# acrlabs/kube-scheduler-rs-reference

Measured on AMD Instinct MI355X. Metric: pod x node predicate evals/s, higher is better.
Workload: dtype int64

## Files before the change

kube_scheduler_rs_reference_amd/csrc/kernels_fused.hpp:

```cpp
#pragma once
#include <hip/hip_ext.h>
#include <hip/hip_runtime.h>
#include <stdint.h>

#include <type_traits>

#include "eval_request.hpp"
#include "kernarg.hpp"
#include "kernels_direct.hpp"
#include "tile_index.hpp"
#include "tile_launch.hpp"

#ifndef KSCHED_STORE_POLICY
#define KSCHED_STORE_POLICY 6
#endif
#ifndef KSCHED_STORE_ALT
#define KSCHED_STORE_ALT(it) ((it) == 7u)
#endif
#ifndef KSCHED_PROFILE
#define KSCHED_PROFILE 0
#endif
#if defined(KSCHED_FUSED_NUM_VGPR)
#define KSCHED_FUSED_WPE_ATTR __attribute__((amdgpu_num_vgpr(KSCHED_FUSED_NUM_VGPR)))
#elif defined(KSCHED_FUSED_WPE)
#define KSCHED_FUSED_WPE_ATTR __attribute__((amdgpu_waves_per_eu(KSCHED_FUSED_WPE, KSCHED_FUSED_WPE)))
#else
#define KSCHED_FUSED_WPE_ATTR
#endif

namespace ksched {

struct FusedArgs {
    uint32_t W, pitch, tiles, rows, nkeys, ngroups;
    uint32_t row_zero, row_valid, row_cpu, row_mem, row_taint;
    uint32_t lab_off[8], lab_mx1[8];
    const uint32_t *lab_meta;
    const uint64_t *zero64;
    uint32_t p, units, chunks, run;
    uint32_t unit_q, unit_rem, tiles_rcp;
    uint32_t wave_major;
    uint32_t u_stride;
    uint32_t off_aux, off_fit, off_lab, off_trow;
    uint32_t nlist, list_mask8, off_list, off_lrec;
    uint32_t list_col[kMaxListKeys];
    uint32_t debug;
    uint32_t has_tol;
    uint32_t pick_ppb, pick_waves;
    uint64_t *pick_acc;
    uint32_t off_park;
    uint32_t off_pf;
    uint64_t *trace;
};

typedef uint32_t u32x4 __attribute__((ext_vector_type(4)));
typedef uint32_t u32x4_a8 __attribute__((ext_vector_type(4), aligned(8)));

template <bool FIT, bool SEL, bool TAINT, bool WANT_FIT, bool LIST = false, int PICK = 0>
__global__ __launch_bounds__(kFusedThreads) KSCHED_FUSED_WPE_ATTR void k_eval_fused(
    const uint64_t *__restrict__ g_tables, const uint64_t *__restrict__ g_aux, const int64_t *__restrict__ g_pcpu,
    const int64_t *__restrict__ g_pmem, const uint32_t *__restrict__ g_psel, const uint64_t *__restrict__ g_ptol,
    uint64_t *__restrict__ out_feas, uint64_t *__restrict__ out_fit, const uint8_t *__restrict__ g_list, const FusedArgs a,
    const SelectArgs sa) {
    static_assert(!LIST || SEL, "list keys only exist with the selector predicate");
    static_assert(!PICK || (!LIST && !WANT_FIT), "the pick rides only in the plain mask variants");
    static_assert(PICK != 2 || !TAINT, "the tile-test pick is built for the reference's two predicates");
    kernarg_warm<9 * 8 + sizeof(FusedArgs) + (PICK ? sizeof(SelectArgs) : 0)>();
    extern __shared__ __attribute__((aligned(16))) uint8_t smem[];
    const uint32_t b = blockIdx.x;
    uint32_t tile, chunk, lin;
    if (!(a.debug & 32u)) {
        const uint32_t l = (b & 7u) * a.run + (b >> 3);
        if ((b >> 3) >= a.run) return;
        chunk = __umulhi(l, a.tiles_rcp);
// ... 9 lines not shown
        lin = chunk * a.tiles + tile;
    }
    if (chunk >= a.chunks) return;

    const uint32_t pick_waves = PICK == 1 ? a.pick_waves : 0u;
    uint32_t tid = threadIdx.x;
    bool pick_wave = false;
    if constexpr (PICK == 1) {
        const uint32_t wave0 = (uint32_t)__builtin_amdgcn_readfirstlane((int)(threadIdx.x >> 6));
        const uint32_t pick_rank = (a.debug & 0x10000u) ? (kFusedWaves - 1u - wave0) : wave0;
        pick_wave = pick_rank < pick_waves;
        if (pick_wave) {
            const uint64_t t_in = (a.trace && threadIdx.x == 0u) ? wall_clock64() : 0ull;
            const uint32_t base = lin * a.pick_ppb;
            const uint32_t end = min(a.p, base + a.pick_ppb);
            const uint32_t eager = (a.debug >> 8) & 3u;
            for (uint32_t pod = base + pick_rank * 64u + (threadIdx.x & 63u); pod < end; pod += pick_waves * 64u) {
                int32_t bnd;
                if (eager == 1u) bnd = select_one_pod<5, 3>(sa, pod);
                else if (eager == 2u) bnd = select_one_pod<5, 5>(sa, pod);
                else if (eager == 3u) bnd = select_one_pod<5, 2>(sa, pod);
                else bnd = select_one_pod<5, 1>(sa, pod);
                sa.binding[pod] = bnd;
            }
            if (a.trace && threadIdx.x == 0u)
                atomicOr((unsigned long long *)&a.trace[(size_t)b * 8u + 7u], (unsigned long long)((wall_clock64() - t_in) << 8));
        }
        asm volatile("" : "+v"(tid) : : "memory");
    }
    const uint32_t lane = tid & 63u;
    const uint32_t wave = __builtin_amdgcn_readfirstlane(tid >> 6);
    const uint32_t stage_rank = (PICK == 1 && !(a.debug & 0x10000u)) ? wave - pick_waves : wave;
    const uint32_t stage_waves = kFusedWaves - pick_waves;
    const bool tracer = a.trace && tid == (PICK == 1 ? (kFusedWaves - 1u) * 64u : 0u);
    auto stamp = [&](uint32_t i) {
        if (tracer) a.trace[(size_t)b * 8u + i] = wall_clock64();
    };
    stamp(0);
    const uint32_t c_lo = chunk * a.unit_q + min(chunk, a.unit_rem);
    const uint32_t c_n = a.unit_q + (chunk < a.unit_rem ? 1u : 0u);
    uint32_t u = c_lo + (wave * c_n) / kFusedWaves;
    uint32_t u_hi = c_lo + ((wave + 1u) * c_n) / kFusedWaves;
    const uint32_t u_stride = a.u_stride;
    if (u_stride != 8u) {
        u = (a.wave_major ? wave * a.chunks + chunk : chunk * kFusedWaves + wave) * 8u;
        u_hi = a.units;
    }

    int64_t rc = 0, rm = 0;
    uint32_t s0 = 0, s1 = 0, s2 = 0, s3 = 0, s4 = 0, s5 = 0, s6 = 0, s7 = 0;
    uint64_t tol = 0;
    uint32_t d0 = 0, d1 = 0, d2 = 0, d3 = 0, d4 = 0;
    uint64_t ar = 0;
    auto issue_ops = [&](uint32_t pod) {
        const uint32_t pc = min(pod, a.p - 1u);
        if constexpr (PICK == 2) {
            static_assert(kPickAttempts == 5, "five draw registers");
            const size_t last = (size_t)a.p * kPickAttempts - 1u;
            const size_t f0 = (size_t)(pod - lane) * kPickAttempts + lane;
            asm volatile("global_load_dword %0, %1, off" : "=v"(d0) : "v"(sa.samples + min(f0, last)) : "memory");
            asm volatile("global_load_dword %0, %1, off" : "=v"(d1) : "v"(sa.samples + min(f0 + 64u, last)) : "memory");
            asm volatile("global_load_dword %0, %1, off" : "=v"(d2) : "v"(sa.samples + min(f0 + 128u, last)) : "memory");
            asm volatile("global_load_dword %0, %1, off" : "=v"(d3) : "v"(sa.samples + min(f0 + 192u, last)) : "memory");
            asm volatile("global_load_dword %0, %1, off" : "=v"(d4) : "v"(sa.samples + min(f0 + 256u, last)) : "memory");
        }
        if (FIT) {
            asm volatile("global_load_dwordx2 %0, %1, off" : "=v"(rc) : "v"(g_pcpu + pc) : "memory");
            asm volatile("global_load_dwordx2 %0, %1, off" : "=v"(rm) : "v"(g_pmem + pc) : "memory");
        }
        if (SEL) {
#define KSCHED_LOAD_SEL(K, DST)                                                                                                   \
    asm volatile("global_load_dword %0, %1, off"                                                                                  \
                 : "=v"(DST)                                                                                                      \
                 : "v"((uint32_t)K < a.nkeys ? g_psel + (size_t)K * a.p + pc : reinterpret_cast<const uint32_t *>(a.zero64)) \
                 : "memory")
            KSCHED_LOAD_SEL(0, s0);
            KSCHED_LOAD_SEL(1, s1);
            KSCHED_LOAD_SEL(2, s2);
            KSCHED_LOAD_SEL(3, s3);
            KSCHED_LOAD_SEL(4, s4);
            KSCHED_LOAD_SEL(5, s5);
            KSCHED_LOAD_SEL(6, s6);
            KSCHED_LOAD_SEL(7, s7);
#undef KSCHED_LOAD_SEL
        }
        if (TAINT) {
            const uint64_t *tp = a.has_tol ? g_ptol + pc : a.zero64;
            asm volatile("global_load_dwordx2 %0, %1, off" : "=v"(tol) : "v"(tp) : "memory");
        }
    };
#define KSCHED_WAIT_OPS(N)                                                                                                            \
    asm volatile("s_waitcnt vmcnt(%c11)"                                                                                              \
                 : "+v"(rc), "+v"(rm), "+v"(s0), "+v"(s1), "+v"(s2), "+v"(s3), "+v"(s4), "+v"(s5), "+v"(s6), "+v"(s7), "+v"(tol)  \
                 : "n"(N)                                                                                                             \
                 : "memory")
#define KSCHED_WAIT_OPS_PICK(N)                                                                                                       \
    asm volatile("s_waitcnt vmcnt(%c17)"                                                                                              \
                 : "+v"(rc), "+v"(rm), "+v"(s0), "+v"(s1), "+v"(s2), "+v"(s3), "+v"(s4), "+v"(s5), "+v"(s6), "+v"(s7), "+v"(tol), \
                   "+v"(d0), "+v"(d1), "+v"(d2), "+v"(d3), "+v"(d4), "+v"(ar)                                                     \
                 : "n"(N)                                                                                                             \
                 : "memory")
    const int64_t *s_cpu = reinterpret_cast<const int64_t *>(smem + a.off_aux);
    const int64_t *s_mem = s_cpu + kAuxTreeWords;
    const uint2 *s_cnt_cpu = reinterpret_cast<const uint2 *>(s_cpu + 2u * kAuxTreeWords);
    const uint2 *s_cnt_mem = s_cnt_cpu + kCntEntries;
    uint4 *s_fit = reinterpret_cast<uint4 *>(smem + a.off_fit) + wave * 64u;
    uint4 *s_lab = reinterpret_cast<uint4 *>(smem + a.off_lab) + wave * 64u;
    uint2 *s_trow = reinterpret_cast<uint2 *>(smem + a.off_trow) + wave * 64u;
    typedef __attribute__((address_space(3))) uint8_t lds_u8;
    lds_u8 *const lds = (lds_u8 *)smem;
    uint2 *s_lrec = reinterpret_cast<uint2 *>(smem + a.off_lrec) + wave * 64u;
    constexpr uint32_t kListCap = 8u;

    const uint32_t quad = (lane & 31u) >> 2;
    const uint32_t wp = ((0xCCu >> quad) & 1u) * 4u + (lane & 3u);
    const uint32_t sub = (lane >> 5) * 4u + ((0x31130220u >> (4u * quad)) & 15u);
    const uint32_t w0 = tile * kTileWords + 2u * wp;
    const bool has0 = w0 < a.pitch, has1 = w0 + 1u < a.pitch;
// ... 133 lines not shown
        const bool live = pod < a.p && has0;
        Rows R;
        if (LIST) {
            uint32_t sub_o = sub, wp_o = wp;
            asm volatile("" : "+v"(sub_o), "+v"(wp_o));
            const uint8_t *fit_o = reinterpret_cast<const uint8_t *>(s_fit + sub_o) + wp_o;
            const uint2 *lab_o = reinterpret_cast<const uint2 *>(s_lab + sub_o);
            load_rows(FIT ? (uint32_t)(fit_o + it * 128u)[0] : 0u, FIT ? (uint32_t)(fit_o + it * 128u)[8] : 0u, (lab_o + it * 16u)[0],
                      TAINT ? (s_trow + sub_o + it * 8u)[0] : make_uint2(0u, 0u), R);
            load_extra((lab_o + it * 16u)[1], R);
        } else {
            load_rows(rec_cc(it), rec_cm(it), rec_lb(it), rec_tr(it), R);
            if (SEL) load_extra(rec_lx(it), R);
        }
        u32x4 f = fit_of(R);
        const size_t o = (size_t)pod * a.pitch + w0;
        auto store = [&](uint64_t *dst) {
            if (has1) store16(dst, o, f);
            else dst[o] = ((uint64_t)f.y << 32) | f.x;
        };
        if (WANT_FIT && live) store(out_fit);
        if (SEL) {
            if (!over) {
                f = ((f & R.l0) & R.l1) & (R.l2 & R.l3);
                f = ((f & R.x0) & R.x1) & (R.x2 & R.x3);
            } else if (live) {
                for (uint32_t k = 0; k < a.nkeys; ++k) {
                    if (LIST && a.lab_meta[k] == kLabList) continue;
                    const uint32_t s = g_psel[(size_t)k * a.p + pod];
                    if (s != 0u) f &= ldrow((s <= a.lab_meta[32u + k]) ? (a.lab_meta[k] + s - 1u) : a.row_zero);
                }
            }
        }
        if (TAINT) {
            if (taint_inline) {
                f = ((f & R.t0) & R.t1) & (R.t2 & R.t3);
            } else if (live) {
                const uint64_t t = a.has_tol ? g_ptol[pod] : 0ull;
                for (uint32_t g = 0; g < a.ngroups; ++g) f &= ldrow(a.row_taint + 16u * g + (uint32_t)((t >> (4u * g)) & 15ull));
            }
        }
        if (LIST) {
            __builtin_amdgcn_sched_barrier(0);
            f = apply_lists(f, lrec_of(it), 0xFFFFFFFFu);
        }
        if (live && out_feas && !(a.debug & 1u)) store(out_feas);
    };

    bool extra_any = false, list_any = false;
    uint32_t list_bound = 0;
    uint32_t pick_bits = 0;
    typedef __attribute__((address_space(3))) uint32_t lds_u32;
    lds_u32 *const s_park = (lds_u32 *)(lds + a.off_park) + wave * (kPickAttempts * 64u);
    auto phase1 = [&](uint32_t pod0) -> uint64_t {
        uint2 cnt_c = make_uint2(0u, 0u), cnt_m = make_uint2(0u, 0u);
        if (FIT) {
            uint32_t lc = 0, lm = 0;
            if (!(a.debug & 2u)) {
                uint32_t kc = 1, km = 1;
#pragma unroll
                for (uint32_t level = 0; level < 10; ++level) {
                    const int64_t vc = s_cpu[kc], vm = s_mem[km];
                    kc = 2u * kc + ((vc < rc) ? 1u : 0u);
                    km = 2u * km + ((vm < rm) ? 1u : 0u);
                }
                lc = kc - (uint32_t)kTileNodes;
                lm = km - (uint32_t)kTileNodes;
                lc += (lc == (uint32_t)kTileNodes - 1u && s_cpu[0] < rc) ? 1u : 0u;
                lm += (lm == (uint32_t)kTileNodes - 1u && s_mem[0] < rm) ? 1u : 0u;
            }
            const uint2 cc = s_cnt_cpu[lc], cm = s_cnt_mem[lm];
            s_fit[lane] = make_uint4(cc.x, cc.y, cm.x, cm.y);
            cnt_c = cc;
            cnt_m = cm;
        }
        const uint32_t rv = a.row_valid * 128u;
        uint32_t cnt = 0;
        if (SEL) {
            const uint32_t rv2 = rv | (rv << 16);
            s_lab[lane] = make_uint4(rv2, rv2, rv2, rv2);
            uint16_t *const slots = reinterpret_cast<uint16_t *>(s_lab + lane);
            uint16_t *slot = slots;
            const uint32_t sv[8] = {s0, s1, s2, s3, s4, s5, s6, s7};
#pragma unroll
            for (uint32_t k = 0; k < 8; ++k) {
                const uint32_t s = sv[k];
                if (s != 0u && !(LIST && ((a.list_mask8 >> k) & 1u))) {
                    *slot++ = (uint16_t)(min(s, a.lab_mx1[k]) * 128u + a.lab_off[k]);
                }
            }
            cnt = (uint32_t)(slot - slots);
            if (a.nkeys > 8u) {
                const uint32_t pc = min(pod0 + lane, a.p - 1u);
                for (uint32_t k = 8; k < a.nkeys; ++k) {
                    if (LIST && a.lab_meta[k] == kLabList) continue;
                    cnt += (g_psel[(size_t)k * a.p + pc] != 0u) ? 9u : 0u;
                }
            }
        }
        uint32_t lmax = 0;
        if (LIST) {
            uint32_t lv[kMaxListKeys] = {0u, 0u};
#pragma unroll
            for (uint32_t j = 0; j < kMaxListKeys; ++j) {
                if (j >= a.nlist) continue;
                const uint32_t col = a.list_col[j];
                if (col < 8u) {
                    uint32_t v = s0;
                    v = (col == 1u) ? s1 : v;
                    v = (col == 2u) ? s2 : v;
                    v = (col == 3u) ? s3 : v;
                    v = (col == 4u) ? s4 : v;
                    v = (col == 5u) ? s5 : v;
                    v = (col == 6u) ? s6 : v;
                    v = (col == 7u) ? s7 : v;
                    lv[j] = v;
                } else {
                    lv[j] = g_psel[(size_t)col * a.p + min(pod0 + lane, a.p - 1u)];
                }
            }
            uint32_t rec[kMaxListKeys] = {0xFFFF0000u, 0xFFFF0000u};
            bool any = false;
#pragma unroll
            for (uint32_t j = 0; j < kMaxListKeys; ++j) {
                rec[j] = 0xFFFF0000u;
                const uint32_t s = lv[j];
                if (j < a.nlist && s != 0u) {
                    const uint32_t voff = a.off_list + j * kListBytes;
                    auto val_at = [&](uint32_t e) -> uint32_t { return *(const __attribute__((address_space(3))) uint32_t *)(lds + voff + e * 4u); };
                    auto lower = [&](uint32_t key) -> uint32_t {
                        uint32_t base = 0;
#pragma unroll
                        for (uint32_t half = (uint32_t)kTileNodes / 2u; half >= 1u; half >>= 1) base += (val_at(base + half - 1u) < key) ? half : 0u;
                        return base + ((val_at(base) < key) ? 1u : 0u);
                    };
                    const uint32_t lo = lower(s);
                    uint32_t cnt = 0;
                    bool run = true;
#pragma unroll
                    for (uint32_t e = 0; e <= kListCap; ++e) {
                        run = run && lo + e < (uint32_t)kTileNodes && val_at(min(lo + e, (uint32_t)kTileNodes - 1u)) == s;
                        cnt += run ? 1u : 0u;
                    }
                    if (cnt > kListCap) cnt = lower(s + 1u) - lo;
                    rec[j] = lo | (cnt << 16);
                    lmax = max(lmax, cnt);
                    any = true;
                }
            }
            s_lrec[lane] = make_uint2(rec[0], rec[1]);
            list_any = __ballot(any) != 0ull;
#pragma unroll
            for (uint32_t d = 32; d >= 1; d >>= 1) lmax = max(lmax, (uint32_t)__shfl_xor((int)lmax, d, 64));
            list_bound = (uint32_t)__builtin_amdgcn_readfirstlane((int)lmax);
        }
        if (TAINT) {
            uint32_t t[4];
#pragma unroll
            for (uint32_t g = 0; g < 4; ++g)
                t[g] = (g < a.ngroups) ? (a.row_taint + 16u * g + (uint32_t)((tol >> (4u * g)) & 15ull)) * 128u : rv;
            s_trow[lane] = make_uint2(t[0] | (t[1] << 16), t[2] | (t[3] << 16));
        }
        if constexpr (PICK == 2) {
            const uint4 slots = SEL ? s_lab[lane] : make_uint4(0u, 0u, 0u, 0u);
            s_park[lane] = d0;
            s_park[64u + lane] = d1;
            s_park[128u + lane] = d2;
            s_park[192u + lane] = d3;
            s_park[256u + lane] = d4;
            uint32_t dv[kPickAttempts];
#pragma unroll
            for (uint32_t i = 0; i < kPickAttempts; ++i) dv[i] = s_park[lane * kPickAttempts + i];
            uint32_t bits = 0;
#pragma unroll
            for (uint32_t i = 0; i < kPickAttempts; ++i) {
                const uint32_t l = dv[i] - tile * (uint32_t)kTileNodes;
                if (l < (uint32_t)kTileNodes && !(a.debug & 0x8000000u)) {
                    const uint32_t wofs = (l >> 5) << 2, sub = l >> 7;
                    auto word = [&](uint32_t off) -> uint32_t { return *(lds_u32 *)(lds + off + wofs); };
                    uint32_t v;
                    if (FIT) {
                        const uint32_t sh = (sub & 3u) * 8u;
                        const uint32_t bc = ((sub < 4u ? cnt_c.x : cnt_c.y) >> sh) & 0xFFu, bm = ((sub < 4u ? cnt_m.x : cnt_m.y) >> sh) & 0xFFu;
                        v = word((a.row_cpu + bc) * 128u) & word((a.row_cpu + (uint32_t)kFitRows + bm) * 128u);
                    } else {
                        v = word(rv);
                    }
                    if (SEL)
                        v &= word(slots.x & 0xFFFFu) & word(slots.x >> 16) & word(slots.y & 0xFFFFu) & word(slots.y >> 16) & word(slots.z & 0xFFFFu) &
                             word(slots.z >> 16) & word(slots.w & 0xFFFFu) & word(slots.w >> 16);
                    bits |= ((v >> (l & 31u)) & 1u) << i;
                }
            }
            pick_bits = bits;
        }
        extra_any = __ballot(cnt > 4u) != 0ull;
        const uint64_t over = __ballot(cnt > 8u || (LIST && lmax > kListCap));
        __builtin_amdgcn_fence(__ATOMIC_RELEASE, "wavefront");
        __builtin_amdgcn_wave_barrier();
        return over;
    };

    constexpr int kFastStores = 8 * (WANT_FIT ? 2 : 1);

    constexpr uint32_t kPrefetchRounds = 6;
    auto prefetch_rounds = [&]() {
        if (!(FIT || SEL || TAINT) || a.off_pf == 0xFFFFFFFFu || u + u_stride * (kPrefetchRounds + 2u) < u_hi || (a.debug & 0x20000000u)) return;
        const uint32_t dump = (uint32_t)__builtin_amdgcn_readfirstlane((int)a.off_pf);
        const uint32_t li = opaque(lane);
#pragma unroll 1
        for (uint32_t r = 1; r <= kPrefetchRounds; ++r) {
            const uint32_t pu = u + u_stride * r;
            if (pu >= u_hi) break;
            const uint32_t pod0 = pu * 8u;
            const uint32_t pe = a.p - 1u;
            const uint32_t e8 = min(pod0 + (li & 3u) * 16u, pe);
            uint64_t a64 = reinterpret_cast<uint64_t>(a.zero64);
            if (FIT && li < 4u) a64 = reinterpret_cast<uint64_t>(g_pcpu + e8);
            if (FIT && li >= 4u && li < 8u) a64 = reinterpret_cast<uint64_t>(g_pmem + e8);
            if (SEL && a.nkeys && li >= 8u && li < 24u) {
                const uint32_t k = min((li - 8u) >> 1, min(a.nkeys, 8u) - 1u);
                a64 = reinterpret_cast<uint64_t>(g_psel + (size_t)k * a.p + min(pod0 + (li & 1u) * 32u, pe));
            }
            if (PICK == 2 && li >= 24u && li < 34u) {
                a64 = reinterpret_cast<uint64_t>(sa.samples + min((size_t)pod0 * kPickAttempts + (li - 24u) * 32u, (size_t)a.p * kPickAttempts - 1u));
            }
            if (TAINT && a.has_tol && li >= 34u && li < 38u) {
                a64 = reinterpret_cast<uint64_t>(g_ptol + e8);
            }
            uint32_t m0_saved;
            asm volatile("s_mov_b32 %0, m0\n\ts_mov_b32 m0, %2\n\ts_nop 0\n\tglobal_load_lds_dword %1, off\n\ts_nop 0\n\ts_mov_b32 m0, %0\n\ts_nop 0" : "=&s"(m0_saved) : "v"(a64), "s"(dump) : "memory");
        }
    };
    bool more = u < u_hi, have_prev = false, first = true, stamped4 = false;
    uint32_t prev_u = 0, prev_nu = 0;
    uint64_t prev_over = 0;
    bool prev_extra = false, prev_list = false;
    uint32_t prev_bound = 0;
#if KSCHED_PROFILE
    uint64_t prof_p2 = 0, prof_wait = 0, prof_p1 = 0, prof_rounds = 0, prof_t = 0;
#define KSCHED_PROF(ACC)                                       \
    do {                                                       \
        const uint64_t now_ = __builtin_readcyclecounter();    \
        ACC += now_ - prof_t;                                  \
        prof_t = now_;                                         \
    } while (0)
#else
#define KSCHED_PROF(ACC) \
    do {                 \
    } while (0)
#endif
    auto pick_contribute = [&](uint32_t pod0, uint32_t nu) {
        const uint32_t n_live = min(nu * 8u, a.p - pod0);
        const uint32_t j = lane & 7u;
        uint32_t lo = 0, hi = 0;
        if (lane < n_live) {
            const uint64_t f = (uint64_t)pick_bits << (5u * j);
            lo = (uint32_t)f;
            hi = (uint32_t)(f >> 32);
        }
#pragma unroll
        for (uint32_t d = 1; d <= 4; d <<= 1) {
            lo |= (uint32_t)__shfl_xor((int)lo, (int)d, 64);
            hi |= (uint32_t)__shfl_xor((int)hi, (int)d, 64);
        }
        const uint64_t delta = (1ull << 40) | ((uint64_t)hi << 32) | (uint64_t)lo;
        uint64_t *const slot = a.pick_acc + ((pod0 >> 3) + (lane >> 3));
        const uint64_t lead = 0x0101010101010101ull & (n_live >= 64u ? ~0ull : ((1ull << n_live) - 1ull));
        uint64_t saved;
        asm volatile("s_and_saveexec_b64 %1, %4\n\tglobal_atomic_add_x2 %0, %2, %3, off sc0\n\ts_mov_b64 exec, %1"
                     : "=v"(ar), "=&s"(saved)
                     : "v"(slot), "v"(delta), "s"(lead)
                     : "memory", "scc");
    };
    auto pick_decide = [&](uint32_t pod0, uint32_t nu) {
        const uint32_t n_live = min(nu * 8u, a.p - pod0);
        const uint32_t j = lane & 7u, first = lane & ~7u;
        const uint32_t wlo = (uint32_t)__shfl((int)(uint32_t)ar, (int)first, 64), whi = (uint32_t)__shfl((int)(uint32_t)(ar >> 32), (int)first, 64);
        const uint64_t word = ((uint64_t)whi << 32) | (uint64_t)wlo;
        if (lane < n_live && (uint32_t)(word >> 40) == a.tiles - 1u) {
            const uint32_t all = ((uint32_t)(word >> (5u * j)) | pick_bits) & ((1u << kPickAttempts) - 1u);
            int32_t bnd = -1;
            if (all) bnd = (int32_t)s_park[lane * kPickAttempts + (uint32_t)__builtin_ctz(all)];
            sa.binding[pod0 + lane] = bnd;
            if (j == 0u) a.pick_acc[(pod0 >> 3) + (lane >> 3)] = 0ull;
        }
    };
    while (true) {
        if (PICK == 2 && have_prev && !(a.debug & 0x10000000u)) pick_contribute(prev_u * 8u, prev_nu);
        if (more) issue_ops(u * 8u + lane);
        if ((a.debug & 128u) && have_prev && !stamped4) stamp(1);
        if (first) {
            auto stage = [&](const void *gsrc, uint32_t lds_off, uint32_t bytes) {
                const uint8_t *g = static_cast<const uint8_t *>(gsrc);
                for (uint32_t off = stage_rank * 1024u; off < bytes; off += stage_waves * 1024u) {
                    if (off + lane * 16u < bytes)
                        __builtin_amdgcn_global_load_lds((const __attribute__((address_space(1))) void *)(g + off + lane * 16u),
                                                         (__attribute__((address_space(3))) void *)(lds + lds_off + off), 16, 0, 0);
                }
            };
            if (!pick_wave) {
                if (FIT) stage(g_aux + (size_t)tile * kAuxWords, a.off_aux, kAuxWords * 8u);
                if (LIST) stage(g_list + (size_t)tile * a.nlist * kListBytes, a.off_list, a.nlist * kListBytes);
                if (!(a.debug & 8u)) stage(g_tables + (size_t)tile * a.rows * kTileWords, 0u, a.rows * 128u);
            }
            if (!(a.debug & 128u)) stamp(1);
            if (PICK == 1) asm volatile("s_waitcnt vmcnt(0)" ::: "memory");
            __syncthreads();
            prefetch_rounds();
            if (!(a.debug & 128u)) stamp(2);
        }
        if (have_prev) {
#if KSCHED_PROFILE
            prof_t = __builtin_readcyclecounter();
#endif
            const uint32_t pod0 = prev_u * 8u;
            rb_feas = uniform64(reinterpret_cast<uint64_t>(out_feas + (size_t)pod0 * a.pitch));
            if (WANT_FIT) rb_fit = uniform64(reinterpret_cast<uint64_t>(out_fit + (size_t)pod0 * a.pitch));
            const bool fast = (prev_nu == 8u || !more) && prev_over == 0ull && pod0 + prev_nu * 8u <= a.p && tile_full &&
                              (!TAINT || taint_inline) && !(a.debug & 16u);
            if (LIST && fast && (prev_list || prev_nu != 8u)) {
                const uint32_t sub_o = opaque(sub), wp_o = opaque(wp);
                const uint8_t *fit_o = reinterpret_cast<const uint8_t *>(s_fit + sub_o) + wp_o;
                const uint2 *lab_o = reinterpret_cast<const uint2 *>(s_lab + sub_o);
                const uint2 *trow_o = s_trow + sub_o;
                Rows A;
                uint2 lr = (s_lrec + sub_o)[0];
                load_rows(FIT ? (uint32_t)fit_o[0] : 0u, FIT ? (uint32_t)fit_o[8] : 0u, lab_o[0], TAINT ? trow_o[0] : make_uint2(0u, 0u), A);
#pragma unroll 1
                for (uint32_t it = 0; it < prev_nu; ++it) {
                    const uint64_t step = (uint64_t)it * step_bytes;
                    u32x4 f = fit_of(A);
                    if (WANT_FIT) store_rel(rb_fit + step, lane_off, f);
                    f = ((f & A.l0) & A.l1) & (A.l2 & A.l3);
                    if (TAINT) f = ((f & A.t0) & A.t1) & (A.t2 & A.t3);
                    if (prev_extra) {
                        load_extra((lab_o + it * 16u)[1], A);
                        f = ((f & A.x0) & A.x1) & (A.x2 & A.x3);
                    }
                    const uint2 lr_now = lr;
                    const uint32_t nx = min(it + 1u, prev_nu - 1u);
                    __builtin_amdgcn_sched_barrier(0);
                    lr = (s_lrec + sub_o + nx * 8u)[0];
// ... 31 lines not shown
                } else {
#pragma unroll
                    for (uint32_t it = 0; it < 8; it += STEP) {
                        Rows R[STEP];
#pragma unroll
                        for (uint32_t j = 0; j < STEP; ++j) load_rows(cn[j], mn[j], ln[j], tn[j], R[j]);
                        if (!TAINT && it + STEP < 8u) {
#pragma unroll
                            for (uint32_t j = 0; j < STEP; ++j) {
                                cn[j] = rec_cc(it + STEP + j);
                                mn[j] = rec_cm(it + STEP + j);
                                ln[j] = rec_lb(it + STEP + j);
                                tn[j] = rec_tr(it + STEP + j);
                            }
                        }
#pragma unroll
                        for (uint32_t j = 0; j < STEP; ++j) combine_store(it + j, R[j], false);
                        if (TAINT && it + STEP < 8u) {
#pragma unroll
                            for (uint32_t j = 0; j < STEP; ++j) {
                                cn[j] = rec_cc(it + STEP + j);
                                mn[j] = rec_cm(it + STEP + j);
                                ln[j] = rec_lb(it + STEP + j);
                                tn[j] = rec_tr(it + STEP + j);
                            }
                        }
                    }
                }
            } else if (!LIST && fast) {
#pragma unroll 1
                for (uint32_t it = 0; it < prev_nu; ++it) {
                    Rows A;
                    load_rows(rec_cc(it), rec_cm(it), rec_lb(it), rec_tr(it), A);
                    if (SEL) load_extra(rec_lx(it), A);
                    combine_store(it, A, true);
                }
            } else {
                if (!(a.debug & 16u)) {
#pragma unroll 1
                    for (uint32_t it = 0; it < prev_nu; ++it) {
                        const uint32_t pl = it * 8u + sub;
                        emit_checked(pod0 + pl, it, (prev_over >> pl) & 1ull);
                    }
                }
                asm volatile("s_waitcnt vmcnt(0)" ::: "memory");
            }
            if (!stamped4) stamp(4);
            stamped4 = true;
            __builtin_amdgcn_fence(__ATOMIC_ACQUIRE, "wavefront");
            __builtin_amdgcn_wave_barrier();
            KSCHED_PROF(prof_p2);
        }
        const bool had_more = more;
        if (more) {
#if KSCHED_PROFILE
            prof_t = __builtin_readcyclecounter();
            ++prof_rounds;
#endif
            if constexpr (PICK == 2) {
                KSCHED_WAIT_OPS_PICK(kFastStores);
                if (have_prev) pick_decide(prev_u * 8u, prev_nu);
            } else {
                KSCHED_WAIT_OPS(kFastStores);
            }
            KSCHED_PROF(prof_wait);
            prev_over = phase1(u * 8u);
            KSCHED_PROF(prof_p1);
            prev_extra = extra_any;
            prev_list = list_any;
            prev_bound = list_bound;
            if (!have_prev) stamp(3);
            prev_u = u;
            prev_nu = min(8u, u_hi - u);
            have_prev = true;
            u += u_stride;
            more = u < u_hi;
        }
        if (PICK == 2 && !had_more && have_prev) {
            asm volatile("s_waitcnt vmcnt(0)" : "+v"(ar) : : "memory");
            pick_decide(prev_u * 8u, prev_nu);
        }
        first = false;
        if (!had_more) break;
    }
#undef KSCHED_WAIT_OPS
#undef KSCHED_WAIT_OPS_PICK
    if (a.trace && lane == 0) {
        atomicMax((unsigned long long *)&a.trace[(size_t)b * 8u + 5u], (unsigned long long)wall_clock64());
        __builtin_amdgcn_s_waitcnt(0);
        atomicMax((unsigned long long *)&a.trace[(size_t)b * 8u + 6u], (unsigned long long)wall_clock64());
    }
#if KSCHED_PROFILE
    if (tracer) {
        a.trace[(size_t)b * 8u + 1u] = prof_p2;
        a.trace[(size_t)b * 8u + 2u] = prof_wait;
        a.trace[(size_t)b * 8u + 3u] = prof_p1;
        a.trace[(size_t)b * 8u + 4u] = prof_rounds;
    }
#endif
#undef KSCHED_PROF
    if (tracer) {
        uint32_t xcc;
        asm volatile("s_getreg_b32 %0, hwreg(HW_REG_XCC_ID)" : "=s"(xcc));
        atomicOr((unsigned long long *)&a.trace[(size_t)b * 8u + 7u], (unsigned long long)(xcc & 0xFFu));
    }
}

struct FusedLaunch {
    dim3 grid;
    uint32_t lds;
    hipStream_t stream;
    const IndexedSnapshot *snap;
    const int64_t *pcpu, *pmem;
    const uint32_t *psel;
    const uint64_t *ptol;
    uint64_t *out_feas, *out_fit;
    hipEvent_t ev_start, ev_stop;
    const SelectArgs *pick;
    int pick_form;
};

template <bool FIT, bool SEL, bool TAINT, bool WANT_FIT, bool LIST, int PICK = 0>
inline hipError_t launch_fused_k(const FusedLaunch &q, const FusedArgs &a) {
    auto kern = k_eval_fused<FIT, SEL, TAINT, WANT_FIT, LIST, PICK>;
    hipError_t e = hipFuncSetAttribute((const void *)kern, hipFuncAttributeMaxDynamicSharedMemorySize, (int)q.lds);
    if (e != hipSuccess) return e;
    const IndexedSnapshot &s = *q.snap;
    const SelectArgs sa = q.pick ? *q.pick : SelectArgs{};
    if (q.ev_start || q.ev_stop)
        hipExtLaunchKernelGGL(kern, q.grid, dim3(kFusedThreads), q.lds, q.stream, q.ev_start, q.ev_stop, 0, s.d_tables, s.d_aux, q.pcpu,
                              q.pmem, q.psel, q.ptol, q.out_feas, q.out_fit, (const uint8_t *)s.d_list, a, sa);
    else
        hipLaunchKernelGGL(kern, q.grid, dim3(kFusedThreads), q.lds, q.stream, s.d_tables, s.d_aux, q.pcpu, q.pmem, q.psel, q.ptol,
                           q.out_feas, q.out_fit, (const uint8_t *)s.d_list, a, sa);
    return hipGetLastError();
}
// ... 77 lines not shown
```

kube_scheduler_rs_reference_amd/csrc/tile_launch.hpp:

```cpp
#pragma once

#include <algorithm>
#include <type_traits>

#include "eval_request.hpp"
#include "tile_index.hpp"

#ifndef KSCHED_FUSED_THREADS
#define KSCHED_FUSED_THREADS 1024
#endif

namespace ksched {

constexpr uint32_t kFusedThreads = KSCHED_FUSED_THREADS;
constexpr uint32_t kFusedWaves = kFusedThreads / 64;

struct TileTerms {
    bool fit, sel, taint;
    bool list;
    bool want_fit;
};

inline TileTerms tile_terms(const EvalRequest &r, const IndexedLayout &l) {
    const bool sel = r.sel(l.nkeys);
// ... 30 lines not shown
    };
    TileLds d{};
    d.off_aux = take(want & kLdsFit, kAuxWords * 8u);
    d.off_fit = take(want & kLdsFit, pods * 16u);
    d.off_lab = take(want & kLdsSel, pods * 16u);
    d.off_trow = take(want & kLdsTaint, pods * 8u);
    d.off_list = take(lists, l.nlist * kListBytes);
    d.off_lrec = take(lists, pods * kListRecBytes);
    d.off_park = take(want & kLdsPark, kPickParkBytes);
    d.off_pf = (want & kLdsPrefetch) && off + kPrefetchDumpBytes <= kLdsBudget ? take(true, kPrefetchDumpBytes) : 0xFFFFFFFFu;
    d.bytes = off;
    return d;
}

constexpr bool lds_is_what_indexed_plan_checks(uint32_t nlist) {
    IndexedLayout l{};
    l.nlist = nlist;
    return tile_lds_layout(l, kLdsEveryRegion).bytes == lds_non_row_bytes(nlist);
}
static_assert(lds_is_what_indexed_plan_checks(0) && lds_is_what_indexed_plan_checks(1) && lds_is_what_indexed_plan_checks(kMaxListKeys),
              "tile_lds_layout and indexed_plan's LDS budget have drifted apart");

inline uint32_t resident_blocks_per_cu(uint32_t lds) { return std::max(1u, std::min(kLdsBudget / lds, 2048u / kFusedThreads)); }

struct FusedGeometryIn {
    uint32_t p = 0, tiles = 1;
    uint32_t lds = 0;
    bool pick = false;
    uint32_t grid_cus = 0;
    int round_order = 0;
    uint32_t debug = 0;
};

struct FusedGeometry {
    uint32_t units, chunks, unit_q, unit_rem;
    uint32_t u_stride, wave_major;
    uint32_t tiles_rcp, run, grid;
    uint32_t pick_ppb, pick_waves;
};

inline FusedGeometry fused_geometry(const FusedGeometryIn &in) {
    FusedGeometry g{};
    g.units = (in.p + 7u) / 8u;
    const uint32_t blocks_per_cu = resident_blocks_per_cu(in.lds);
    const uint32_t rounds = (g.units + 7u) / 8u;
    uint32_t per_block = kFusedWaves;
    if (in.pick) per_block = 4u;
    if (((in.debug >> 18) & 3u) == 1u) per_block = kFusedWaves;
    if (((in.debug >> 18) & 3u) == 2u) per_block = 4u;
    if (((in.debug >> 18) & 3u) == 3u) per_block = 1u;
    const uint32_t want = (rounds + per_block - 1u) / per_block;
    const uint32_t cus = in.grid_cus ? std::min(256u, in.grid_cus) : 256u;
    g.chunks = std::max(1u, std::min((cus * blocks_per_cu) / in.tiles, want));
    if (in.round_order != 1 && !(in.debug & 0x80000000u)) {
        const uint32_t streams = g.chunks * kFusedWaves;
        const uint32_t per_wave = (rounds + streams - 1u) / streams;
        if (per_wave == 2u) g.chunks = std::max(1u, std::min(g.chunks, (rounds + 2u * kFusedWaves - 1u) / (2u * kFusedWaves)));
    }
    g.unit_q = g.units / g.chunks;
    g.unit_rem = g.units % g.chunks;
    g.u_stride = in.round_order == 1 ? 8u : g.chunks * kFusedWaves * 8u;
    g.wave_major = in.round_order == 2 ? 0u : 1u;
    g.tiles_rcp = (uint32_t)std::min<uint64_t>((1ull << 32) / in.tiles, 0xFFFFFFFFull);
    const uint32_t total = g.chunks * in.tiles;
    g.run = (total + 7u) / 8u;
    g.grid = (in.debug & 32u) ? total : g.run * 8u;
    if (in.pick) {
        g.pick_ppb = (in.p + total - 1u) / total;
        g.pick_waves = std::max(1u, std::min(8u, (g.pick_ppb + 63u) / 64u));
    }
    return g;
}

struct SummaryGeometry {
    uint32_t rounds, chunks, grid;
};

inline SummaryGeometry summary_geometry(uint32_t p, uint32_t tiles, uint32_t lds) {
    SummaryGeometry g{};
    g.rounds = (p + 63u) / 64u;
    g.chunks = std::max(1u, std::min((256u * resident_blocks_per_cu(lds)) / tiles, (g.rounds + kFusedWaves - 1u) / kFusedWaves));
    g.grid = g.chunks * tiles;
    return g;
}

template <class Args>
inline void fill_tile_args(Args &a, const IndexedSnapshot &s, const TileLds &d, const TileTerms &t, const EvalRequest &r) {
    const IndexedLayout &l = s.lay;
    a.p = r.p;
    a.tiles = l.tiles;
    a.rows = l.rows;
    a.nkeys = l.nkeys;
    a.ngroups = l.ngroups;
    a.row_zero = l.row_zero;
    a.row_valid = l.row_valid;
    a.row_cpu = l.row_cpu;
    a.row_taint = l.row_taint;
    for (int k = 0; k < 8; ++k) {
        const bool is_list = l.lab_base[k] == kLabList;
        a.lab_off[k] = is_list ? 0u : (l.lab_base[k] - 1u) * 128u;
        a.lab_mx1[k] = is_list ? 0u : l.lab_max[k] + 1u;
    }
    a.lab_meta = s.d_lab_meta;
    a.zero64 = reinterpret_cast<const uint64_t *>(s.d_lab_meta + 64);
    a.off_aux = d.off_aux;
    a.off_fit = d.off_fit;
// ... 21 lines not shown
```

Measured before the change: 25530 billion.

## Defer pick draw loads and tests one round behind predicate stores

Adds a default-on mode where, for the PICK==2 path, the random-draw sample loads, the pick tests and the pick contribution are run one round behind the main predicate work. The draw loads are issued for the previous unit, and the pick decision for the unit before that. The prefetch loop and the loop exit are adjusted to drain the extra stage. The aim is to hide draw-load latency and the pick work behind the feasibility stores. In exchange the pipeline is deeper, needs more bookkeeping state and an extra drain iteration, and may use more registers. A debug bit that forces a single chunk is also added.

```diff
diff --git a/kube_scheduler_rs_reference_amd/csrc/kernels_fused.hpp b/kube_scheduler_rs_reference_amd/csrc/kernels_fused.hpp
--- a/kube_scheduler_rs_reference_amd/csrc/kernels_fused.hpp
+++ b/kube_scheduler_rs_reference_amd/csrc/kernels_fused.hpp
@@ -19,6 +19,9 @@
 #endif
 #ifndef KSCHED_PROFILE
 #define KSCHED_PROFILE 0
+#endif
+#ifndef KSCHED_PICK_BEHIND_STORES
+#define KSCHED_PICK_BEHIND_STORES 1
 #endif
 #if defined(KSCHED_FUSED_NUM_VGPR)
 #define KSCHED_FUSED_WPE_ATTR __attribute__((amdgpu_num_vgpr(KSCHED_FUSED_NUM_VGPR)))
@@ -134,8 +137,8 @@
     uint64_t tol = 0;
     uint32_t d0 = 0, d1 = 0, d2 = 0, d3 = 0, d4 = 0;
     uint64_t ar = 0;
-    auto issue_ops = [&](uint32_t pod) {
-        const uint32_t pc = min(pod, a.p - 1u);
+    constexpr bool kBehind = PICK == 2 && KSCHED_PICK_BEHIND_STORES;
+    auto issue_draws = [&](uint32_t pod) {
         if constexpr (PICK == 2) {
             static_assert(kPickAttempts == 5, "five draw registers");
             const size_t last = (size_t)a.p * kPickAttempts - 1u;
@@ -146,6 +149,10 @@
             asm volatile("global_load_dword %0, %1, off" : "=v"(d3) : "v"(sa.samples + min(f0 + 192u, last)) : "memory");
             asm volatile("global_load_dword %0, %1, off" : "=v"(d4) : "v"(sa.samples + min(f0 + 256u, last)) : "memory");
         }
+    };
+    auto issue_ops = [&](uint32_t pod) {
+        const uint32_t pc = min(pod, a.p - 1u);
+        if constexpr (PICK == 2 && !kBehind) issue_draws(pod);
         if (FIT) {
             asm volatile("global_load_dwordx2 %0, %1, off" : "=v"(rc) : "v"(g_pcpu + pc) : "memory");
             asm volatile("global_load_dwordx2 %0, %1, off" : "=v"(rm) : "v"(g_pmem + pc) : "memory");
@@ -385,117 +392,9 @@
     uint32_t pick_bits = 0;
     typedef __attribute__((address_space(3))) uint32_t lds_u32;
     lds_u32 *const s_park = (lds_u32 *)(lds + a.off_park) + wave * (kPickAttempts * 64u);
-    auto phase1 = [&](uint32_t pod0) -> uint64_t {
-        uint2 cnt_c = make_uint2(0u, 0u), cnt_m = make_uint2(0u, 0u);
-        if (FIT) {
-            uint32_t lc = 0, lm = 0;
-            if (!(a.debug & 2u)) {
-                uint32_t kc = 1, km = 1;
-#pragma unroll
-                for (uint32_t level = 0; level < 10; ++level) {
-                    const int64_t vc = s_cpu[kc], vm = s_mem[km];
-                    kc = 2u * kc + ((vc < rc) ? 1u : 0u);
-                    km = 2u * km + ((vm < rm) ? 1u : 0u);
-                }
-                lc = kc - (uint32_t)kTileNodes;
-                lm = km - (uint32_t)kTileNodes;
-                lc += (lc == (uint32_t)kTileNodes - 1u && s_cpu[0] < rc) ? 1u : 0u;
-                lm += (lm == (uint32_t)kTileNodes - 1u && s_mem[0] < rm) ? 1u : 0u;
-            }
-            const uint2 cc = s_cnt_cpu[lc], cm = s_cnt_mem[lm];
-            s_fit[lane] = make_uint4(cc.x, cc.y, cm.x, cm.y);
-            cnt_c = cc;
-            cnt_m = cm;
-        }
-        const uint32_t rv = a.row_valid * 128u;
-        uint32_t cnt = 0;
-        if (SEL) {
-            const uint32_t rv2 = rv | (rv << 16);
-            s_lab[lane] = make_uint4(rv2, rv2, rv2, rv2);
-            uint16_t *const slots = reinterpret_cast<uint16_t *>(s_lab + lane);
-            uint16_t *slot = slots;
-            const uint32_t sv[8] = {s0, s1, s2, s3, s4, s5, s6, s7};
-#pragma unroll
-            for (uint32_t k = 0; k < 8; ++k) {
-                const uint32_t s = sv[k];
-                if (s != 0u && !(LIST && ((a.list_mask8 >> k) & 1u))) {
-                    *slot++ = (uint16_t)(min(s, a.lab_mx1[k]) * 128u + a.lab_off[k]);
-                }
-            }
-            cnt = (uint32_t)(slot - slots);
-            if (a.nkeys > 8u) {
-                const uint32_t pc = min(pod0 + lane, a.p - 1u);
-                for (uint32_t k = 8; k < a.nkeys; ++k) {
-                    if (LIST && a.lab_meta[k] == kLabList) continue;
-                    cnt += (g_psel[(size_t)k * a.p + pc] != 0u) ? 9u : 0u;
-                }
-            }
-        }
-        uint32_t lmax = 0;
-        if (LIST) {
-            uint32_t lv[kMaxListKeys] = {0u, 0u};
-#pragma unroll
-            for (uint32_t j = 0; j < kMaxListKeys; ++j) {
-                if (j >= a.nlist) continue;
-                const uint32_t col = a.list_col[j];
-                if (col < 8u) {
-                    uint32_t v = s0;
-                    v = (col == 1u) ? s1 : v;
-                    v = (col == 2u) ? s2 : v;
-                    v = (col == 3u) ? s3 : v;
-                    v = (col == 4u) ? s4 : v;
-                    v = (col == 5u) ? s5 : v;
-                    v = (col == 6u) ? s6 : v;
-                    v = (col == 7u) ? s7 : v;
-                    lv[j] = v;
-                } else {
-                    lv[j] = g_psel[(size_t)col * a.p + min(pod0 + lane, a.p - 1u)];
-                }
-            }
-            uint32_t rec[kMaxListKeys] = {0xFFFF0000u, 0xFFFF0000u};
-            bool any = false;
-#pragma unroll
-            for (uint32_t j = 0; j < kMaxListKeys; ++j) {
-                rec[j] = 0xFFFF0000u;
-                const uint32_t s = lv[j];
-                if (j < a.nlist && s != 0u) {
-                    const uint32_t voff = a.off_list + j * kListBytes;
-                    auto val_at = [&](uint32_t e) -> uint32_t { return *(const __attribute__((address_space(3))) uint32_t *)(lds + voff + e * 4u); };
-                    auto lower = [&](uint32_t key) -> uint32_t {
-                        uint32_t base = 0;
-#pragma unroll
-                        for (uint32_t half = (uint32_t)kTileNodes / 2u; half >= 1u; half >>= 1) base += (val_at(base + half - 1u) < key) ? half : 0u;
-                        return base + ((val_at(base) < key) ? 1u : 0u);
-                    };
-                    const uint32_t lo = lower(s);
-                    uint32_t cnt = 0;
-                    bool run = true;
-#pragma unroll
-                    for (uint32_t e = 0; e <= kListCap; ++e) {
-                        run = run && lo + e < (uint32_t)kTileNodes && val_at(min(lo + e, (uint32_t)kTileNodes - 1u)) == s;
-                        cnt += run ? 1u : 0u;
-                    }
-                    if (cnt > kListCap) cnt = lower(s + 1u) - lo;
-                    rec[j] = lo | (cnt << 16);
-                    lmax = max(lmax, cnt);
-                    any = true;
-                }
-            }
-            s_lrec[lane] = make_uint2(rec[0], rec[1]);
-            list_any = __ballot(any) != 0ull;
-#pragma unroll
-            for (uint32_t d = 32; d >= 1; d >>= 1) lmax = max(lmax, (uint32_t)__shfl_xor((int)lmax, d, 64));
-            list_bound = (uint32_t)__builtin_amdgcn_readfirstlane((int)lmax);
-        }
-        if (TAINT) {
-            uint32_t t[4];
-#pragma unroll
-            for (uint32_t g = 0; g < 4; ++g)
-                t[g] = (g < a.ngroups) ? (a.row_taint + 16u * g + (uint32_t)((tol >> (4u * g)) & 15ull)) * 128u : rv;
-            s_trow[lane] = make_uint2(t[0] | (t[1] << 16), t[2] | (t[3] << 16));
-        }
+    auto pick_tests = [&](const uint2 cnt_c, const uint2 cnt_m, const uint4 slots) -> uint32_t {
         if constexpr (PICK == 2) {
-            const uint4 slots = SEL ? s_lab[lane] : make_uint4(0u, 0u, 0u, 0u);
+            const uint32_t rv = a.row_valid * 128u;
             s_park[lane] = d0;
             s_park[64u + lane] = d1;
             s_park[128u + lane] = d2;
@@ -525,8 +424,121 @@
                     bits |= ((v >> (l & 31u)) & 1u) << i;
                 }
             }
-            pick_bits = bits;
-        }
+            return bits;
+        }
+        return 0u;
+    };
+    auto phase1 = [&](uint32_t pod0) -> uint64_t {
+        uint2 cnt_c = make_uint2(0u, 0u), cnt_m = make_uint2(0u, 0u);
+        if (FIT) {
+            uint32_t lc = 0, lm = 0;
+            if (!(a.debug & 2u)) {
+                uint32_t kc = 1, km = 1;
+#pragma unroll
+                for (uint32_t level = 0; level < 10; ++level) {
+                    const int64_t vc = s_cpu[kc], vm = s_mem[km];
+                    kc = 2u * kc + ((vc < rc) ? 1u : 0u);
+                    km = 2u * km + ((vm < rm) ? 1u : 0u);
+                }
+                lc = kc - (uint32_t)kTileNodes;
+                lm = km - (uint32_t)kTileNodes;
+                lc += (lc == (uint32_t)kTileNodes - 1u && s_cpu[0] < rc) ? 1u : 0u;
+                lm += (lm == (uint32_t)kTileNodes - 1u && s_mem[0] < rm) ? 1u : 0u;
+            }
+            const uint2 cc = s_cnt_cpu[lc], cm = s_cnt_mem[lm];
+            s_fit[lane] = make_uint4(cc.x, cc.y, cm.x, cm.y);
+            cnt_c = cc;
+            cnt_m = cm;
+        }
+        const uint32_t rv = a.row_valid * 128u;
+        uint32_t cnt = 0;
+        if (SEL) {
+            const uint32_t rv2 = rv | (rv << 16);
+            s_lab[lane] = make_uint4(rv2, rv2, rv2, rv2);
+            uint16_t *const slots = reinterpret_cast<uint16_t *>(s_lab + lane);
+            uint16_t *slot = slots;
+            const uint32_t sv[8] = {s0, s1, s2, s3, s4, s5, s6, s7};
+#pragma unroll
+            for (uint32_t k = 0; k < 8; ++k) {
+                const uint32_t s = sv[k];
+                if (s != 0u && !(LIST && ((a.list_mask8 >> k) & 1u))) {
+                    *slot++ = (uint16_t)(min(s, a.lab_mx1[k]) * 128u + a.lab_off[k]);
+                }
+            }
+            cnt = (uint32_t)(slot - slots);
+            if (a.nkeys > 8u) {
+                const uint32_t pc = min(pod0 + lane, a.p - 1u);
+                for (uint32_t k = 8; k < a.nkeys; ++k) {
+                    if (LIST && a.lab_meta[k] == kLabList) continue;
+                    cnt += (g_psel[(size_t)k * a.p + pc] != 0u) ? 9u : 0u;
+                }
+            }
+        }
+        uint32_t lmax = 0;
+        if (LIST) {
+            uint32_t lv[kMaxListKeys] = {0u, 0u};
+#pragma unroll
+            for (uint32_t j = 0; j < kMaxListKeys; ++j) {
+                if (j >= a.nlist) continue;
+                const uint32_t col = a.list_col[j];
+                if (col < 8u) {
+                    uint32_t v = s0;
+                    v = (col == 1u) ? s1 : v;
+                    v = (col == 2u) ? s2 : v;
+                    v = (col == 3u) ? s3 : v;
+                    v = (col == 4u) ? s4 : v;
+                    v = (col == 5u) ? s5 : v;
+                    v = (col == 6u) ? s6 : v;
+                    v = (col == 7u) ? s7 : v;
+                    lv[j] = v;
+                } else {
+                    lv[j] = g_psel[(size_t)col * a.p + min(pod0 + lane, a.p - 1u)];
+                }
+            }
+            uint32_t rec[kMaxListKeys] = {0xFFFF0000u, 0xFFFF0000u};
+            bool any = false;
+#pragma unroll
+            for (uint32_t j = 0; j < kMaxListKeys; ++j) {
+                rec[j] = 0xFFFF0000u;
+                const uint32_t s = lv[j];
+                if (j < a.nlist && s != 0u) {
+                    const uint32_t voff = a.off_list + j * kListBytes;
+                    auto val_at = [&](uint32_t e) -> uint32_t { return *(const __attribute__((address_space(3))) uint32_t *)(lds + voff + e * 4u); };
+                    auto lower = [&](uint32_t key) -> uint32_t {
+                        uint32_t base = 0;
+#pragma unroll
+                        for (uint32_t half = (uint32_t)kTileNodes / 2u; half >= 1u; half >>= 1) base += (val_at(base + half - 1u) < key) ? half : 0u;
+                        return base + ((val_at(base) < key) ? 1u : 0u);
+                    };
+                    const uint32_t lo = lower(s);
+                    uint32_t cnt = 0;
+                    bool run = true;
+#pragma unroll
+                    for (uint32_t e = 0; e <= kListCap; ++e) {
+                        run = run && lo + e < (uint32_t)kTileNodes && val_at(min(lo + e, (uint32_t)kTileNodes - 1u)) == s;
+                        cnt += run ? 1u : 0u;
+                    }
+                    if (cnt > kListCap) cnt = lower(s + 1u) - lo;
+                    rec[j] = lo | (cnt << 16);
+                    lmax = max(lmax, cnt);
+                    any = true;
+                }
+            }
+            s_lrec[lane] = make_uint2(rec[0], rec[1]);
+            list_any = __ballot(any) != 0ull;
+#pragma unroll
+            for (uint32_t d = 32; d >= 1; d >>= 1) lmax = max(lmax, (uint32_t)__shfl_xor((int)lmax, d, 64));
+            list_bound = (uint32_t)__builtin_amdgcn_readfirstlane((int)lmax);
+        }
+        if (TAINT) {
+            uint32_t t[4];
+#pragma unroll
+            for (uint32_t g = 0; g < 4; ++g)
+                t[g] = (g < a.ngroups) ? (a.row_taint + 16u * g + (uint32_t)((tol >> (4u * g)) & 15ull)) * 128u : rv;
+            s_trow[lane] = make_uint2(t[0] | (t[1] << 16), t[2] | (t[3] << 16));
+        }
+        if constexpr (PICK == 2 && !kBehind)
+            pick_bits = pick_tests(cnt_c, cnt_m, SEL ? s_lab[lane] : make_uint4(0u, 0u, 0u, 0u));
         extra_any = __ballot(cnt > 4u) != 0ull;
         const uint64_t over = __ballot(cnt > 8u || (LIST && lmax > kListCap));
         __builtin_amdgcn_fence(__ATOMIC_RELEASE, "wavefront");
@@ -544,19 +556,26 @@
 #pragma unroll 1
         for (uint32_t r = 1; r <= kPrefetchRounds; ++r) {
             const uint32_t pu = u + u_stride * r;
-            if (pu >= u_hi) break;
+            bool ops_round = true;
+            if constexpr (kBehind) {
+                ops_round = pu < u_hi;
+                if (!ops_round && pu - u_stride >= u_hi) break;
+            } else {
+                if (pu >= u_hi) break;
+            }
             const uint32_t pod0 = pu * 8u;
             const uint32_t pe = a.p - 1u;
             const uint32_t e8 = min(pod0 + (li & 3u) * 16u, pe);
             uint64_t a64 = reinterpret_cast<uint64_t>(a.zero64);
-            if (FIT && li < 4u) a64 = reinterpret_cast<uint64_t>(g_pcpu + e8);
-            if (FIT && li >= 4u && li < 8u) a64 = reinterpret_cast<uint64_t>(g_pmem + e8);
-            if (SEL && a.nkeys && li >= 8u && li < 24u) {
+            if (FIT && (!kBehind || ops_round) && li < 4u) a64 = reinterpret_cast<uint64_t>(g_pcpu + e8);
+            if (FIT && (!kBehind || ops_round) && li >= 4u && li < 8u) a64 = reinterpret_cast<uint64_t>(g_pmem + e8);
+            if (SEL && (!kBehind || ops_round) && a.nkeys && li >= 8u && li < 24u) {
                 const uint32_t k = min((li - 8u) >> 1, min(a.nkeys, 8u) - 1u);
                 a64 = reinterpret_cast<uint64_t>(g_psel + (size_t)k * a.p + min(pod0 + (li & 1u) * 32u, pe));
             }
             if (PICK == 2 && li >= 24u && li < 34u) {
-                a64 = reinterpret_cast<uint64_t>(sa.samples + min((size_t)pod0 * kPickAttempts + (li - 24u) * 32u, (size_t)a.p * kPickAttempts - 1u));
+                const uint32_t pod0d = kBehind ? pod0 - u_stride * 8u : pod0;
+                a64 = reinterpret_cast<uint64_t>(sa.samples + min((size_t)pod0d * kPickAttempts + (li - 24u) * 32u, (size_t)a.p * kPickAttempts - 1u));
             }
             if (TAINT && a.has_tol && li >= 34u && li < 38u) {
                 a64 = reinterpret_cast<uint64_t>(g_ptol + e8);
@@ -619,9 +638,13 @@
             if (j == 0u) a.pick_acc[(pod0 >> 3) + (lane >> 3)] = 0ull;
         }
     };
+    bool have_pp = false;
+    uint32_t pp_u = 0, pp_nu = 0;
     while (true) {
-        if (PICK == 2 && have_prev && !(a.debug & 0x10000000u)) pick_contribute(prev_u * 8u, prev_nu);
+        if (PICK == 2 && !kBehind && have_prev && !(a.debug & 0x10000000u)) pick_contribute(prev_u * 8u, prev_nu);
         if (more) issue_ops(u * 8u + lane);
+        if constexpr (kBehind)
+            if (have_prev) issue_draws(prev_u * 8u + lane);
         if ((a.debug & 128u) && have_prev && !stamped4) stamp(1);
         if (first) {
             auto stage = [&](const void *gsrc, uint32_t lds_off, uint32_t bytes) {
@@ -759,12 +782,29 @@
             KSCHED_PROF(prof_p2);
         }
         const bool had_more = more;
+        if constexpr (kBehind) {
+            if (more || have_prev || have_pp) {
+                if (!more && !(have_prev && prev_nu == 8u)) asm volatile("s_waitcnt vmcnt(0)" ::: "memory");
+                KSCHED_WAIT_OPS_PICK(kFastStores);
+                if (have_pp) pick_decide(pp_u * 8u, pp_nu);
+                have_pp = false;
+                if (have_prev) {
+                    const uint4 fr = FIT ? s_fit[lane] : make_uint4(0u, 0u, 0u, 0u);
+                    pick_bits = pick_tests(make_uint2(fr.x, fr.y), make_uint2(fr.z, fr.w), SEL ? s_lab[lane] : make_uint4(0u, 0u, 0u, 0u));
+                    if (!(a.debug & 0x10000000u)) pick_contribute(prev_u * 8u, prev_nu);
+                    pp_u = prev_u;
+                    pp_nu = prev_nu;
+                    have_pp = true;
+                }
+            }
+        }
         if (more) {
 #if KSCHED_PROFILE
             prof_t = __builtin_readcyclecounter();
             ++prof_rounds;
 #endif
-            if constexpr (PICK == 2) {
+            if constexpr (kBehind) {
+            } else if constexpr (PICK == 2) {
                 KSCHED_WAIT_OPS_PICK(kFastStores);
                 if (have_prev) pick_decide(prev_u * 8u, prev_nu);
             } else {
@@ -783,12 +823,19 @@
             u += u_stride;
             more = u < u_hi;
         }
-        if (PICK == 2 && !had_more && have_prev) {
+        if (PICK == 2 && !kBehind && !had_more && have_prev) {
             asm volatile("s_waitcnt vmcnt(0)" : "+v"(ar) : : "memory");
             pick_decide(prev_u * 8u, prev_nu);
         }
         first = false;
-        if (!had_more) break;
+        if constexpr (kBehind) {
+            if (!had_more) {
+                if (!have_pp) break;
+                have_prev = false;
+            }
+        } else {
+            if (!had_more) break;
+        }
     }
 #undef KSCHED_WAIT_OPS
 #undef KSCHED_WAIT_OPS_PICK
diff --git a/kube_scheduler_rs_reference_amd/csrc/tile_launch.hpp b/kube_scheduler_rs_reference_amd/csrc/tile_launch.hpp
--- a/kube_scheduler_rs_reference_amd/csrc/tile_launch.hpp
+++ b/kube_scheduler_rs_reference_amd/csrc/tile_launch.hpp
@@ -106,6 +106,7 @@
     const uint32_t want = (rounds + per_block - 1u) / per_block;
     const uint32_t cus = in.grid_cus ? std::min(256u, in.grid_cus) : 256u;
     g.chunks = std::max(1u, std::min((cus * blocks_per_cu) / in.tiles, want));
+    if (in.debug & 0x20000u) g.chunks = 1u;
     if (in.round_order != 1 && !(in.debug & 0x80000000u)) {
         const uint32_t streams = g.chunks * kFusedWaves;
         const uint32_t per_wave = (rounds + streams - 1u) / streams;
```

New measurement: 24910 billion. -2.4%, worse.
